# 4ment/physher

Hardware: AMD Instinct MI355X
Metric: lnL+gradient evals/sec, 1000-taxon GTR+G4 fp64, 1e6 site patterns (higher is better)
Workload: dtype f64

## Files before the change

include/physher_amd.h:

```cpp
#ifndef PHYSHER_AMD_H
#define PHYSHER_AMD_H

#include <stddef.h>
#include <stdint.h>

#ifdef __cplusplus
extern "C" {
#endif

typedef struct phyamd_engine phyamd_engine;

enum {
	PHYAMD_OK = 0,
	PHYAMD_EINVAL = -1,
	PHYAMD_EDEVICE = -2,
	PHYAMD_ENOMEM = -3,
	PHYAMD_EUNSUPPORTED = -4
};

enum { PHYAMD_RESCALE_NEVER = 0, PHYAMD_RESCALE_ALWAYS = 1, PHYAMD_RESCALE_AUTO = 2 };

enum {
	PHYAMD_GRAD_FOLD_ROOT_FREQS = 1,
	PHYAMD_GRAD_COMPAT_SCALED = 2
// ... 91 lines not shown
                                         double *replicate_lnl );
typedef struct { int32_t items, chunks, replicate_chunks, lower_slots; int64_t scratch_bytes; double ms; } phyamd_site_lnl_profile;
int phyamd_get_site_lnl_profile(phyamd_engine *e, phyamd_site_lnl_profile *out);
int phyamd_synchronize(phyamd_engine *e);

int phyamd_get_pattern_log_likelihoods(phyamd_engine *e, double *out );
int phyamd_get_partials(phyamd_engine *e, int node, int upper, double *out);
int phyamd_get_node_matrices(phyamd_engine *e, int node, int derivative, double *out );
int phyamd_post_order_parks(int32_t tip_count, const int32_t *left , const int32_t *right, int32_t root, int32_t second_slot,
                            int32_t *out , int32_t capacity);
#define PHYAMD_PRE_ORDER_COLUMNS 30
int phyamd_pre_order_schedule(int32_t tip_count, const int32_t *left , const int32_t *right, int32_t root, int32_t form,
                              int32_t *out , int32_t capacity, int32_t *hbm_slots);
int phyamd_post_order_slots(int32_t tip_count, const int32_t *left , const int32_t *right, int32_t root,
                            int32_t *out , int32_t capacity, int32_t *slots);
int phyamd_is_rescaling(phyamd_engine *e);
int phyamd_set_rescaling(phyamd_engine *e, int policy);
int phyamd_set_keep_partials(phyamd_engine *e, int on);

typedef struct {
	double matrices_ms, lower_ms, upper_ms, reduce_ms;
	int32_t lower_launches, upper_launches;
	int64_t device_bytes;
	int32_t tiles;
} phyamd_profile;
int phyamd_set_reduction_levels(phyamd_engine *e, int levels);
int phyamd_set_profiling(phyamd_engine *e, int on);
int phyamd_get_profile(phyamd_engine *e, phyamd_profile *out);

#ifdef __cplusplus
// ... 4 lines not shown
```

physher_amd/_lib.py:

```python
from __future__ import annotations

import ctypes as C
import os

_HERE = os.path.dirname(os.path.abspath(__file__))
LIB_PATH = os.environ.get("PHYAMD_LIB") or os.path.join(_HERE, "libphysher_amd.so")

ABI_VERSION = 5

OK, EINVAL, EDEVICE, ENOMEM, EUNSUPPORTED = 0, -1, -2, -3, -4
RESCALE_NEVER, RESCALE_ALWAYS, RESCALE_AUTO = 0, 1, 2
GRAD_FOLD_ROOT_FREQS, GRAD_COMPAT_SCALED = 1, 2


class Config(C.Structure):
    _fields_ = [
        ("tip_count", C.c_int32), ("pattern_count", C.c_int32), ("state_count", C.c_int32),
        ("category_count", C.c_int32), ("device", C.c_int32), ("rescale", C.c_int32),
        ("max_device_bytes", C.c_int64), ("stream", C.c_void_p),
    ]


class Profile(C.Structure):
    _fields_ = [
# ... 84 lines not shown
    ("phyamd_site_rate_posteriors", C.c_int, [_P, _P, _P]),
    ("phyamd_branch_hessian", C.c_int, [_P, C.c_int, _P, _P, _P]),
    ("phyamd_get_hessian_profile", C.c_int, [_P, C.POINTER(HessianProfile)]),
    ("phyamd_get_general_profile", C.c_int, [_P, C.POINTER(GeneralProfile)]),
    ("phyamd_gradient_batch_weights", C.c_int, [_P, C.c_int, C.c_int32, _P, _P, _P, _P]),
    ("phyamd_get_weight_batch_profile", C.c_int, [_P, C.POINTER(WeightBatchProfile)]),
    ("phyamd_pattern_log_likelihoods_trees", C.c_int, [_P, C.c_int, C.c_int32, _P, _P, _P, _P, _P, _P, C.c_int32, _P, _P]),
    ("phyamd_get_site_lnl_profile", C.c_int, [_P, C.POINTER(SiteLnlProfile)]),
    ("phyamd_synchronize", C.c_int, [_P]),
    ("phyamd_get_pattern_log_likelihoods", C.c_int, [_P, _P]),
    ("phyamd_get_partials", C.c_int, [_P, C.c_int, C.c_int, _P]),
    ("phyamd_get_node_matrices", C.c_int, [_P, C.c_int, C.c_int, _P]),
    ("phyamd_post_order_parks", C.c_int, [C.c_int32, _P, _P, C.c_int32, C.c_int32, _P, C.c_int32]),
    ("phyamd_post_order_slots", C.c_int, [C.c_int32, _P, _P, C.c_int32, _P, C.c_int32, _P]),
    ("phyamd_pre_order_schedule", C.c_int, [C.c_int32, _P, _P, C.c_int32, C.c_int32, _P, C.c_int32, _P]),
    ("phyamd_is_rescaling", C.c_int, [_P]),
    ("phyamd_set_rescaling", C.c_int, [_P, C.c_int]),
    ("phyamd_set_keep_partials", C.c_int, [_P, C.c_int]),
    ("phyamd_set_reduction_levels", C.c_int, [_P, C.c_int]),
    ("phyamd_set_profiling", C.c_int, [_P, C.c_int]),
    ("phyamd_get_profile", C.c_int, [_P, C.POINTER(Profile)]),
    ("phyamd_store", C.c_int, [_P]),
    ("phyamd_restore", C.c_int, [_P]),
    ("phyamd_compress_patterns", C.c_int, [C.c_int, C.c_int32, C.c_int64, _P, _P, C.POINTER(C.c_int32), _P, _P]),
]

_lib = None


def load():
# ... 21 lines not shown
```

physher_amd/csrc/phyamd_abi.inc:

```

#include <condition_variable>
#include <functional>
#include <mutex>
#include <thread>

namespace {

class ShardWorkers {
public:
	explicit ShardWorkers(int n) : done_(0), generation_(0), stop_(false) {
		for (int i = 0; i < n; i++) threads_.emplace_back([this, i] { loop(i); });
	}
	~ShardWorkers() {
		{
			std::lock_guard<std::mutex> lk(m_);
			stop_ = true;
			generation_++;
		}
		cv_.notify_all();
		for (auto &t : threads_) t.join();
	}
	void run(const std::function<void(int)> &fn) {
		std::unique_lock<std::mutex> lk(m_);
		fn_ = &fn;
// ... 820 lines not shown
			rec[18] = o.carry_out;
			const int kl = o.kind_left, kr = o.kind_right;
			const int rows[10] = {o.left, o.right, kl >= CH_CHERRY ? o.lt0 : -1, kl >= CH_CHERRY ? o.lt1 : -1, kl == CH_CHERRY_TIP ? o.linner : -1,
			                      kl == CH_CHERRY_TIP ? o.lt2 : -1, kr >= CH_CHERRY ? o.rt0 : -1, kr >= CH_CHERRY ? o.rt1 : -1,
			                      kr == CH_CHERRY_TIP ? o.rinner : -1, kr == CH_CHERRY_TIP ? o.rt2 : -1};
			for (int j = 0; j < 10; j++)
				if (rows[j] >= 0) q[nq++] = rows[j];
		}
		rec[17] = (is_cut_root[rec[2]] ? 1 : 0) | (is_cut_root[rec[3]] ? 2 : 0);
		rec[19] = nq;
		std::memcpy(out + (size_t)i * W, rec, sizeof(rec));
	}
	return (int)ops.size();
}

int phyamd_is_rescaling(phyamd_engine *g) {
	CHECK_GROUP(g);
	int any = 0;
	for (Shard *s : g->shards) any |= shard_is_rescaling(s);
	return any;
}

int phyamd_get_profile(phyamd_engine *g, phyamd_profile *out) {
	CHECK_GROUP(g);
	if (!out) return fail(PHYAMD_EINVAL, "null out");
	int rc;
	if ((rc = shard_get_profile(g->shards[0], out))) return rc;
	for (int i = 1; i < group_size(g); i++) {
		phyamd_profile p;
		if ((rc = shard_get_profile(g->shards[i], &p))) return rc;
// ... 12 lines not shown
```

physher_amd/csrc/phyamd_launch.inc:

```

size_t gen_image_doubles(const Shard *e) {
	return e->S == 20 ? MatImage<2, 5>::SIZE : e->S == 60 ? MatImage<4, 15>::SIZE : MatImage<4, 16>::SIZE;
}

template <int RT, int KT>
void launch_matrix_images(Shard *e, int count, const double *src, double *dst, const double *rowscale) {
	hipLaunchKernelGGL((k_matrix_images<RT, KT>), dim3(count), dim3(256), 0, e->stream, e->S, src, dst, rowscale);
}

void build_matrix_images(Shard *e, int count, const double *src, double *dst, const double *rowscale = nullptr) {
	if (e->S == 20) launch_matrix_images<2, 5>(e, count, src, dst, rowscale);
	else if (e->S == 60) launch_matrix_images<4, 15>(e, count, src, dst, rowscale);
	else launch_matrix_images<4, 16>(e, count, src, dst, rowscale);
}

int update_matrices(Shard *e) {
	if (e->generic && e->state.qimg_dirty && e->have_Q && e->have_freqs) {
		build_matrix_images(e, 1, e->d_Q, e->d_imgs + (size_t)e->N * e->C * gen_image_doubles(e));
		build_matrix_images(e, 1, e->d_Q, e->d_imgs + ((size_t)e->N * e->C + 1) * gen_image_doubles(e), e->d_freqs);
		HIP_TRY(hipGetLastError());
		q_images_rebuilt(e);
	}
	if (!e->state.matrices_dirty) return PHYAMD_OK;
	if (e->have_eigen) {
// ... 390 lines not shown
	if (v.scale < 0) return fail(PHYAMD_EDEVICE, "streamed walk: the stored lowers hold the %s form, which no %s post-order pass writes", form_name(e->lower_form), SCALE ? "rescaled" : "plain");
	const bool exp2 = v.scale == 2, tf = v.tf;
	if (exp2 && (rc = e->d_uexp.ensure(std::max<size_t>(1, upper_slots_held(e)) * e->C * e->P))) return rc;
	const int waves = SCALE && !exp2 ? e->C : STREAM_WAVES;
	const size_t lds = (size_t)STREAM_LDS_PER_WAVE * waves + (exp2 ? (size_t)waves * STREAM_PARK_SLOTS * WAVE * sizeof(int) : SCALE ? (size_t)4 * e->C * WAVE * sizeof(double) : 0);
	const dim3 grid_x(SCALE && !exp2 ? (unsigned)nb : (unsigned)((nb + STREAM_WAVES - 1) / STREAM_WAVES) * e->C), block(WAVE, waves);
	hipLaunchKernelGGL(k_op_tables, dim3(nops, e->C), dim3(64), 0, e->stream, nops, e->C, (const int *)e->d_stream_op_tips, (const int *)e->d_stream_op_deep,
	                   (const int *)e->d_stream_site_tab, e->d_mats, FOLD ? e->d_Q : e->d_Qpi, reinterpret_cast<double *>(e->d_optab.get()));
	const int subtrees = (int)e->sched.walk_chunk_off.size() - 2;
	for (int phase = 0; phase < (subtrees > 0 ? 2 : 1); phase++) {
		const bool amb = e->stream_ambiguous;
		auto *kernel = exp2 ? (amb ? k_upper4_stream<FOLD, 2, true, true> : k_upper4_stream<FOLD, 2, false, true>)
		             : SCALE ? (amb ? k_upper4_stream<FOLD, 1, true, false> : k_upper4_stream<FOLD, 1, false, false>)
		             : tf    ? (amb ? k_upper4_stream<FOLD, 0, true, true> : k_upper4_stream<FOLD, 0, false, true>)
		                     : (amb ? k_upper4_stream<FOLD, 0, true, false> : k_upper4_stream<FOLD, 0, false, false>);
		hipLaunchKernelGGL(kernel, dim3(grid_x.x, phase ? subtrees : 1), block, lds, e->stream, (const StreamDesc *)e->d_stream_ops, (const StreamChunk *)e->d_stream_chunks,
		                   (const int *)e->d_walk_chunk_off, phase, nops, e->P, e->C, nb, (const uint32_t *)e->d_mstream, e->mstride, (const double *)e->d_lower, e->d_upper,
		                   (const double *)e->d_mats, (const char *)e->d_optab, (const double *)(FOLD ? e->d_Q : e->d_Qpi), (const double *)e->d_freqs, (const double *)e->d_wl,
		                   e->d_gslab, R, (const double *)e->d_props, (const double *)e->d_weights, e->xcd_map, (const int *)e->d_lexp, e->d_uexp, (const int *)e->d_Eroot);
	}
	HIP_TRY(hipGetLastError());
	e->prof.upper_launches = subtrees > 0 ? 2 : 1;
	e->grad_blocks = nb;
	e->slab_walk_order = true;
	return PHYAMD_OK;
}

void bisect_blocks(int lo, int hi, int levels, std::vector<int> &bounds) {
	if (levels == 0) {
		bounds.push_back(lo);
		return;
// ... 404 lines not shown
```

physher_amd/csrc/phyamd_schedule.inc:

```

int bind_device(Shard *e) {
	HIP_TRY(hipSetDevice(e->device));
	return PHYAMD_OK;
}

size_t node_partial_doubles(const Shard *e) { return (size_t)e->C * e->S * (e->generic ? e->Pp : e->P); }
size_t lower_slots(const Shard *e) { return e->d_lower.size() / node_partial_doubles(e); }
size_t upper_slots_held(const Shard *e) { return e->d_upper.size() / node_partial_doubles(e); }

int ensure_lower_storage(Shard *e) {
	const size_t need = (size_t)std::max(1, e->sched.core_count) * (e->two_slots ? 2 : 1);
	if (lower_slots(e) >= need) return PHYAMD_OK;
	e->d_lower.release();
	e->d_lscale.release();
	return e->d_lower.ensure(need * node_partial_doubles(e));
}

void refresh_op_cores(Schedule &s) {
	for (std::vector<NodeOp> *ops : {&s.lower_ops, &s.upper_ops, &s.walk_lower_ops, &s.walk_upper_ops, &s.walk_chunk_ops, &s.walk_lower_chunk_ops})
		for (NodeOp &op : *ops) {
			op.core_parent = s.core_index[op.parent];
			op.core_left = s.core_index[op.left];
			op.core_right = s.core_index[op.right];
		}
// ... 9 lines not shown
		HIP_TRY(hipMemcpyAsync(e->d_tiptab + (size_t)e->T * e->C * 64, e->sched.deep_host.data(), e->sched.deep_host.size() * sizeof(DeepDesc), hipMemcpyHostToDevice,
		                       e->stream));
	if (e->sched.walking || e->sched.gen_walking) {
		if ((rc = e->d_walk_lower_ops.ensure(e->N)) || (rc = e->d_walk_upper_ops.ensure(e->N))) return rc;
		HIP_TRY(hipMemcpyAsync(e->d_walk_lower_ops, e->sched.walk_lower_ops.data(), e->sched.walk_lower_ops.size() * sizeof(NodeOp), hipMemcpyHostToDevice, e->stream));
		HIP_TRY(hipMemcpyAsync(e->d_walk_upper_ops, e->sched.walk_upper_ops.data(), e->sched.walk_upper_ops.size() * sizeof(NodeOp), hipMemcpyHostToDevice, e->stream));
	}
	if (e->sched.walking) {
		if ((rc = e->d_walk_chunk_ops.ensure(e->N)) || (rc = e->d_walk_chunk_off.ensure((size_t)e->N + 2))) return rc;
		HIP_TRY(hipMemcpyAsync(e->d_walk_chunk_ops, e->sched.walk_chunk_ops.data(), e->sched.walk_chunk_ops.size() * sizeof(NodeOp), hipMemcpyHostToDevice, e->stream));
		HIP_TRY(hipMemcpyAsync(e->d_walk_chunk_off, e->sched.walk_chunk_off.data(), e->sched.walk_chunk_off.size() * sizeof(int), hipMemcpyHostToDevice, e->stream));
		if ((rc = e->d_walk_lower_chunk_ops.ensure(e->N)) || (rc = e->d_walk_lower_chunk_off.ensure((size_t)e->N + 2))) return rc;
		HIP_TRY(hipMemcpyAsync(e->d_walk_lower_chunk_ops, e->sched.walk_lower_chunk_ops.data(), e->sched.walk_lower_chunk_ops.size() * sizeof(NodeOp), hipMemcpyHostToDevice, e->stream));
		HIP_TRY(hipMemcpyAsync(e->d_walk_lower_chunk_off, e->sched.walk_lower_chunk_off.data(), e->sched.walk_lower_chunk_off.size() * sizeof(int), hipMemcpyHostToDevice, e->stream));
		if (stream_possible(e)) {
			build_stream_tables(e->sched, StreamGeometry{e->P, e->C, (size_t)e->nblk_walk_upper * e->G * WAVE}, &e->stream_tab);
			if ((rc = e->d_stream_ops.ensure(e->N)) || (rc = e->d_stream_chunks.ensure((size_t)e->N + 2)) || (rc = e->d_stream_row_entries.ensure((size_t)e->N * 32)) ||
			    (rc = e->d_stream_site_tab.ensure((size_t)e->N * 16)) || (rc = e->d_stream_qnode.ensure(e->N)) || (rc = e->d_stream_op_tips.ensure((size_t)e->N * 12)) ||
			    (rc = e->d_stream_flag.ensure(1)) || (rc = e->d_stream_op_deep.ensure(e->N)))
				return rc;
			HIP_TRY(hipMemcpyAsync(e->d_stream_op_tips, e->stream_tab.op_tips.data(), e->stream_tab.op_tips.size() * sizeof(int), hipMemcpyHostToDevice, e->stream));
			HIP_TRY(hipMemcpyAsync(e->d_stream_op_deep, e->stream_tab.op_deep.data(), e->stream_tab.op_deep.size() * sizeof(int), hipMemcpyHostToDevice, e->stream));
			HIP_TRY(hipMemcpyAsync(e->d_stream_ops, e->stream_tab.desc.data(), e->stream_tab.desc.size() * sizeof(StreamDesc), hipMemcpyHostToDevice, e->stream));
			HIP_TRY(hipMemcpyAsync(e->d_stream_chunks, e->stream_tab.chunks.data(), e->stream_tab.chunks.size() * sizeof(StreamChunk), hipMemcpyHostToDevice, e->stream));
			HIP_TRY(hipMemcpyAsync(e->d_stream_row_entries, e->stream_tab.row_entries.data(), e->stream_tab.row_entries.size() * sizeof(int), hipMemcpyHostToDevice, e->stream));
			HIP_TRY(hipMemcpyAsync(e->d_stream_site_tab, e->stream_tab.site_tab.data(), e->stream_tab.site_tab.size() * sizeof(int), hipMemcpyHostToDevice, e->stream));
			HIP_TRY(hipMemcpyAsync(e->d_stream_qnode, e->stream_tab.qnode.data(), e->stream_tab.qnode.size() * sizeof(int), hipMemcpyHostToDevice, e->stream));
			if ((rc = e->d_lstream_ops.ensure(e->N)) || (rc = e->d_lstream_chunks.ensure((size_t)e->N + 2))) return rc;
			HIP_TRY(hipMemcpyAsync(e->d_lstream_ops, e->stream_tab.lower_desc.data(), e->stream_tab.lower_desc.size() * sizeof(LowerDesc), hipMemcpyHostToDevice, e->stream));
			HIP_TRY(hipMemcpyAsync(e->d_lstream_chunks, e->stream_tab.lower_chunks.data(), e->stream_tab.lower_chunks.size() * sizeof(LowerChunk), hipMemcpyHostToDevice, e->stream));
		}
	}
	std::vector<uint8_t> valid((size_t)e->N * e->C, 1);
	for (int c = 0; c < e->C; c++) valid[(size_t)e->root * e->C + c] = 0;
	HIP_TRY(hipMemcpyAsync(e->d_row_valid, valid.data(), valid.size(), hipMemcpyHostToDevice, e->stream));
	HIP_TRY(hipStreamSynchronize(e->stream));
	return PHYAMD_OK;
}

// ... 27 lines not shown
```

physher_amd/csrc/phyamd_shard.inc:

```

enum class LowerForm { Reference, Carried, CarriedExp2 };

struct ScheduleCounts { int core_count, upper_slots, widest; };

struct Shard {
	phyamd_config cfg{};
	DeviceBudget mem;
	DeviceBudget tile_mem{&mem};
	int T = 0, N = 0, P = 0, S = 0, C = 0, root = -1;
	int G = 1;
	bool generic = false;
	int Pp = 0;
	int nblk_root = 0;
	int nblk_lower = 0;
	int nblk_walk = 0, nblk_walk_upper = 0;
	int lower_walk_slots[2] = {0, 0};
	int gen_slots[3][2] = {};
	int lnl_blocks = 0;
	int grad_blocks = 0;
	size_t gpart_row = 0;
	struct State {
		bool all_dirty = true;
		std::vector<int> changed;
		bool force_root = false;
// ... 67 lines not shown
	int device = 0;
	hipStream_t stream = nullptr;
	bool own_stream = false;

	std::vector<int32_t> left, right;
	std::vector<double> lengths, model, freqs, rates, props;
	std::vector<double> lengths_sent;
	std::vector<uint8_t> explicit_host;
	bool have_topology = false, have_lengths = false, have_eigen = false, have_freqs = false, have_rates = false, have_weights = false;
	std::vector<uint8_t> tip_set;
	bool scaling_on = false;
	LowerForm lower_form = LowerForm::Reference;
	bool reference_form_only = false;
	bool exp2_on = true, tform_on = true;
	bool lower_park2_on = true;
	DeviceArray<int> d_lexp{&tile_mem}, d_uexp{&tile_mem}, d_Ec{&tile_mem}, d_Eroot{&tile_mem};
	bool keep_partials = false;
	bool profiling = false;
	bool prof_pending = false, prof_with_upper = false;

	Schedule sched;
	Schedule sched_spare;
	StreamTables stream_tab;
	ScheduleCounts scaled_counts{0, 0, 1};
	bool have_scaled_counts = false;
	bool fusion_enabled = true;

	DeviceArray<uint8_t> d_tipmask{&tile_mem};
	DeviceArray<unsigned long long> d_tipsets{&mem};
	std::vector<unsigned long long> tipsets_host;
// ... 238 lines not shown
```

physher_amd/csrc/phyamd_shard_api.inc:

```

ScheduleCounts schedule_counts(const Schedule &s) {
	ScheduleCounts c{s.core_count, std::max(s.upper_slots, s.walk_upper_slots), 1};
	for (size_t i = 0; i + 1 < s.lower_level_off.size(); i++) c.widest = std::max(c.widest, s.lower_level_off[i + 1] - s.lower_level_off[i]);
	for (size_t i = 0; i + 1 < s.upper_level_off.size(); i++) c.widest = std::max(c.widest, s.upper_level_off[i + 1] - s.upper_level_off[i]);
	return c;
}

double tile_working_set(const Shard *e, double p, bool exact, const ScheduleCounts &k) {
	const double pp = e->S == 4 ? p : std::ceil(p / 16.0) * 16.0, npd = (double)e->C * e->S * pp;
	const double per_pattern = (double)e->T * p + 8.0 * p * (3.0 + (e->S == 4 ? 0.0 : (double)e->C));
	const bool may_scale = e->cfg.rescale != PHYAMD_RESCALE_NEVER, exponents = may_scale && e->S == 4 && e->exp2_on;
	if (!exact) return 8.0 * (exponents ? 1.125 : 1.0) * ((e->S == 4 ? 0.5 : 1.6) * (double)(e->N - e->T) * npd + 2.0 * npd) + per_pattern;
	double doubles = (double)(std::max(1, k.core_count) + std::max(1, k.upper_slots)) * npd;
	if (may_scale) doubles += (double)std::max(1, k.core_count) * p + (e->S == 4 ? 0.0 : 5.0 * k.widest * e->C * p);
	if (exponents) doubles += 0.5 * ((double)(std::max(1, k.core_count) + std::max(1, k.upper_slots) + 1) * e->C * p + p);
	if (e->S == 4) doubles += (double)e->C * p;
	doubles += (double)e->N * e->C * (p / (WAVE * std::max(1, 4 / e->C)) + 1.0);
	if (e->S == 4) doubles += 2.0 * e->N * (p / (WAVE * PPT_UPPER) + 19.0) + 0.5 * p / 64.0;
	return 8.0 * doubles + per_pattern;
}

double tile_working_set(const Shard *e, double p, bool exact) {
	const double now = tile_working_set(e, p, exact, schedule_counts(e->sched));
	return e->have_scaled_counts ? std::max(now, tile_working_set(e, p, exact, e->scaled_counts)) : now;
// ... 135 lines not shown
	if ((rc = choose_tiles(e, false))) return bail(rc);
	if (cfg->stream) e->stream = (hipStream_t)cfg->stream;
	else {
		hipError_t err = hipStreamCreateWithFlags(&e->stream, hipStreamNonBlocking);
		if (err != hipSuccess) return bail(fail(PHYAMD_EDEVICE, "hipStreamCreate: %s", hipGetErrorString(err)));
		e->own_stream = true;
	}
	e->scaling_on = cfg->rescale == PHYAMD_RESCALE_ALWAYS;
	if (const char *env = std::getenv("PHYAMD_FUSE")) e->fusion_enabled = std::atoi(env) != 0;
	if (const char *env = std::getenv("PHYAMD_WALK")) e->walk_enabled = std::atoi(env) != 0;
	if (const char *env = std::getenv("PHYAMD_GEN_FUSION")) e->generic_fusion = std::atoi(env) != 0;
	if (const char *env = std::getenv("PHYAMD_XCD_MAP")) e->xcd_map = std::atoi(env) != 0;
	if (const char *env = std::getenv("PHYAMD_SCALE_EXP2")) e->exp2_on = std::atoi(env) != 0;
	if (const char *env = std::getenv("PHYAMD_STREAM_TFORM")) e->tform_on = std::atoi(env) != 0;
	if (const char *env = std::getenv("PHYAMD_LOWER_PARK2")) e->lower_park2_on = std::atoi(env) != 0;
	e->generic = e->S != 4;
	e->tip_set.assign(e->T, 0);
	e->tip_empty.assign(e->T, 0);
	e->mem.spare = &e->batch_mem;
	e->batch_max_patterns = BATCH_MAX_PATTERNS;
	if (const char *env = std::getenv("PHYAMD_BATCH_MAX_PATTERNS")) e->batch_max_patterns = std::atoi(env);
	if (const char *env = std::getenv("PHYAMD_BATCH_TRACE")) e->batch_trace = std::atoi(env) != 0;
	e->explicit_host.assign(e->N, 0);
	const size_t msz = (size_t)e->N * e->C * e->S * e->S;
	if (e->generic && ((rc = e->d_tipsets.ensure(256)) || (rc = e->d_imgs.ensure(((size_t)e->N * e->C + 2) * gen_image_doubles(e))))) return bail(rc);
	if (e->S == 20 && GenFuse<2>::QP) {
		if ((rc = e->d_qp_mats.ensure((size_t)e->T * e->C * e->S * e->S)) || (rc = e->d_qp_imgs.ensure((size_t)e->T * e->C * gen_image_doubles(e)))) return bail(rc);
	}
	if ((rc = e->d_mats.ensure(msz)) || (rc = e->d_dmats.ensure(msz)) || (rc = e->d_model.ensure((size_t)e->S + 2 * e->S * e->S)) ||
	    (rc = e->d_Q.ensure((size_t)e->S * e->S)))
// ... 895 lines not shown
```

physher_amd/csrc/phyamd_tree_schedule.h:

```cpp
#ifndef PHYAMD_TREE_SCHEDULE_H
#define PHYAMD_TREE_SCHEDULE_H

#include <algorithm>
#include <cstdarg>
#include <cstdint>
#include <cstdio>
#include <string>
#include <utility>
#include <vector>

#include "phyamd_types.h"

struct TreeRef {
	int T;
	const int32_t *left, *right;
	int root;
};

inline std::string schedule_error(const char *fmt, ...) {
	char buf[512];
	va_list ap;
	va_start(ap, fmt);
	vsnprintf(buf, sizeof buf, fmt, ap);
	va_end(ap);
// ... 525 lines not shown
		sc.walk_lower_ops.reserve(tree.T - 1);
		sc.walk_upper_ops.reserve(tree.T - 1);
		b.walk_post_order();
		b.walk_pre_order();
		if (sc.walking) {
			chunk_pre_order(sc);
			chunk_post_order(sc);
		}
	}
	return std::string();
}

struct StreamGeometry {
	int P, C;
	size_t mstride;
};

struct StreamTables {
	std::vector<StreamOp> ops;
	std::vector<StreamDesc> desc;
	int P = 0;
	size_t mstride = 0;
	std::vector<StreamChunk> chunks;
	std::vector<LowerDesc> lower_desc;
	std::vector<LowerChunk> lower_chunks;
	std::vector<int> row_entries;
	std::vector<int> site_tab;
	std::vector<int> qnode;
	std::vector<int> op_tips;
	std::vector<int> op_deep;
	int words = 0, R = 0;
};

struct MaskPacker {
	std::vector<int> &rows;
	int row = -1, used = 32, entries = 8;
	explicit MaskPacker(std::vector<int> &r) : rows(r), row((int)r.size() / 8 - 1) {}
	void add(const int *tips, int &out_row, int &out_shift) {
		int span = 0, n = 0;
		for (int j = 0; j < 6; j++)
			if (tips[j] >= 0) {
				span = j + 1;
				n++;
			}
		const int bits = 1 + 4 * span;
// ... 285 lines not shown
			const bool last = i + 1 == en;
			const int sn = last ? 0 : sop[sc.walk_lower_chunk_ops[i + 1].parent];
			d.nx_block = sn;
			int first = 0;
			const int count = last ? 0 : fresh_rows(i + 1, first);
			d.nx_words = (int64_t)first * row_bytes;
			d.flags |= count << 14;
			d.flags |= (first & 3) << 12;
			d.flags |= (last ? 0 : ((pieces[i + 1] & 2) ? 1 : 0)) << 24;
			d.flags |= (last ? 0 : (pieces[i + 1] & 1)) << 25;
		}
	}
	t.words = (int)t.row_entries.size() / 8;
}

inline void build_stream_tables(const Schedule &sc, const StreamGeometry &g, StreamTables *out) {
	stream_pre_order(sc, g, *out);
	stream_post_order(sc, g, *out);
}


inline int build_batch_ops(int T, const int32_t *left, const int32_t *right, int root, std::vector<BatchOp> *ops, bool park_all = false) {
	const int N = 2 * T - 1;
	std::vector<int> size(N, 1), order;
	{
		std::vector<int> stack{root};
		while (!stack.empty()) {
			const int n = stack.back();
			stack.pop_back();
			order.push_back(n);
			if (n >= T) {
				stack.push_back(left[n]);
				stack.push_back(right[n]);
// ... 99 lines not shown
```

physher_amd/csrc/phyamd_types.h:

```cpp
#ifndef PHYAMD_TYPES_H
#define PHYAMD_TYPES_H

#include <cstddef>
#include <cstdint>

constexpr int WAVE = 64;

enum { CH_TIP = 0, CH_CORE = 1, CH_DEEP = 2, CH_CHERRY = 3, CH_CHERRY_TIP = 4 };

struct DeepDesc {
	int32_t kind_left, left, lt0, lt1, lt2, linner;
	int32_t kind_right, right, rt0, rt1, rt2, rinner;
};

struct NodeOp {
	int32_t parent;
	int32_t left, right;
	int32_t upper_slot_parent;
	int32_t upper_slot_left, upper_slot_right;
	int32_t core_parent, core_left, core_right;
	int32_t kind_left, kind_right;
	int32_t lt0, lt1, lt2, linner;
	int32_t rt0, rt1, rt2, rinner;
	int32_t carry_in;
// ... 1 lines not shown
	int32_t lds_park;
};

constexpr int WALK_CHUNKS = 3;

struct BatchOp {
	int32_t node, left, right;
	int32_t carry;
	int32_t src, dst_left, dst_right;
	int32_t pad;
};
enum { BATCH_NONE = -1, BATCH_CARRY = -2, BATCH_ROOT = -3, BATCH_GHOST = -4 };

enum { HK_TIP = 0, HK_CHERRY = 1, HK_CHERRY_TIP = 2 };
enum { SU_CARRY = 0, SU_LDS = 1, SU_U = 2, SU_ROOT = 3 };

struct StreamOp {
	int32_t flags;
	int32_t parent;
	int32_t slot_parent, slot_left, slot_right;
	int32_t nx_mask_word;
	int32_t nx_a, nx_b;
	int32_t lnode, la[10];
	int32_t rnode, ra[10];
	int32_t nx_u;
	int32_t wsh;
};
static_assert(sizeof(StreamOp) == 128, "one StreamOp = 32 dwords");

struct StreamDesc {
// ... 39 lines not shown
```

physher_amd/csrc/phyamd_walk4s.inc:

```


__global__ __launch_bounds__(256) void k_build_mask_stream(int rows, int P, size_t mstride, const int *__restrict__ row_entries, const uint8_t *__restrict__ tipmask,
                                                           uint32_t *__restrict__ mstream, int *__restrict__ flags) {
	const size_t k = (size_t)blockIdx.x * 256 + threadIdx.x;
	if (k >= mstride) return;
	bool bad = false, amb = false;
	for (int w = blockIdx.y; w < rows; w += gridDim.y) {
		uint32_t v = 0;
		for (int j = 0; j < 8; j++) {
			const int ent = row_entries[w * 8 + j];
			if (ent < 0) continue;
			const int t = ent & 0xFFFFF, pos = (ent >> 20) & 31, fpos = (ent >> 25) & 31;
			const uint32_t m = (k < (size_t)P ? tipmask[(size_t)t * P + k] : 0xFu) & 0xFu;
			const uint32_t code = m == 1 ? 0 : m == 2 ? 1 : m == 4 ? 2 : m == 8 ? 3 : (m == 15 || m == 0) ? 4 : m == 3 ? 5 : m < 8 ? m + 1 : m;
			bad |= m == 0;
			if (code >= 5) {
				amb = true;
				v |= 1u << fpos;
			}
			v |= code << pos;
		}
		mstream[(size_t)w * mstride + k] = v;
	}
	if (bad || amb) atomicOr(flags, (bad ? 1 : 0) | (amb ? 2 : 0));
// ... 102 lines not shown
	template <int A, int R, bool FIRST = false>
	__device__ __forceinline__ void add_tip(const d4 &u, const d4 &qb) {
		put<A, R, FIRST>(dot4(u, qb));
	}
};

template <int SIDE, bool KEEP_BN>
__device__ __forceinline__ d4 s_fringe_message(const SX &x, int kind, int node, int inner, unsigned w, d4 &bn) {
	d4 p = mul4(x.site_tip<SIDE, 0>(w), x.site_tip<SIDE, 1>(w));
	if (kind == CH_CHERRY_TIP) {
		const d4 inner_message = matvec4_opt<false>(x.M(inner), p);
		if (KEEP_BN) bn = inner_message;
		p = mul4(inner_message, x.site_tip<SIDE, 2>(w));
	}
	return matvec4_opt<false>(x.M(node), p);
}

template <int SIDE, bool FIRST2, bool KEEP_BN, typename SS>
__device__ __forceinline__ void s_descend(const SX &x, SS &ss, int kind, int node, int inner, const d4 &u, unsigned w, const d4 &bn_kept) {
	d4 a2 = matvec4_opt<false>(x.M(node), u);
	if (kind == CH_CHERRY_TIP) {
		const d4 bn = KEEP_BN ? bn_kept : matvec4_opt<false>(x.M(inner), mul4(x.site_tip<SIDE, 0>(w), x.site_tip<SIDE, 1>(w)));
		const d4 un = mul4(a2, x.site_tip<SIDE, 2>(w));
		ss.template add<SIDE, 3>(un, bn);
		ss.template add_tip<2, SIDE, FIRST2>(mul4(a2, bn), x.site_tip_q<SIDE, 2>(w));
		a2 = matvec4_opt<false>(x.M(inner), un);
	}
	ss.template add_tip<SIDE, 1>(mul4(a2, x.site_tip<SIDE, 1>(w)), x.site_tip_q<SIDE, 0>(w));
	ss.template add_tip<SIDE, 2>(mul4(a2, x.site_tip<SIDE, 0>(w)), x.site_tip_q<SIDE, 1>(w));
}
// ... 211 lines not shown
		} else if (usrc == SU_U) {
			ea = eU;
			a = matvec4_opt<false>(x.M(op.parent), U);
			if (!SCALE && !valid) a = d4{0., 0., 0., 0.};
		}
		else a = FOLD ? d4{wl * freqs[0], wl * freqs[1], wl * freqs[2], wl * freqs[3]} : d4{wl, wl, wl, wl};
		d4 bl, br, bnl, bnr;
		if (KEEP_BN) {
			any_value(bnl);
			any_value(bnr);
		}
		if (kl == CH_CORE) bl = TF ? own_registers(A) : matvec4_opt<false>(x.M(op.lnode), A);
		else if (kl == CH_TIP) bl = x.site_tip<0, 0>(wL);
		else if (kl == CH_DEEP)
			bl = matvec4_opt<false>(x.M(op.lnode), mul4(s_half<0, 0>(x, (fl >> 16) & 3, op.lm[0], op.lm[1], wL), s_half<0, 3>(x, (fl >> 18) & 3, op.lm[2], op.lm[3], wL)));
		else bl = s_fringe_message<0, KEEP_BN>(x, kl, op.lnode, op.lm[4], wL, bnl);
		if (kr == CH_CORE) br = TF ? own_registers(B) : matvec4_opt<false>(x.M(op.rnode), B);
		else if (kr == CH_TIP) br = x.site_tip<1, 0>(wR);
		else if (kr == CH_DEEP)
			br = matvec4_opt<false>(x.M(op.rnode), mul4(s_half<1, 0>(x, (fl >> 20) & 3, op.rm[0], op.rm[1], wR), s_half<1, 3>(x, (fl >> 22) & 3, op.rm[2], op.rm[3], wR)));
		else br = s_fringe_message<1, KEEP_BN>(x, kr, op.rnode, op.rm[4], wR, bnr);
		const int e_bl = EXP2 && kl == CH_CORE ? eA : 0, e_br = EXP2 && kr == CH_CORE ? eB : 0;
		__builtin_amdgcn_s_setprio(3);
		unsigned nw0 = 0, nw1 = 0;
		if (i + 1 < op_end) fetch_block(i + 1, (fl >> 24) & 1);
		if (nxw > 0) nw0 = word_at(op.nx_words);
		if (nxw > 1) nw1 = word_at(op.nx_words + ((fl >> 25) & 1 ? (int64_t)0 : (int64_t)mrow));
		if (fl & (1 << 26)) A = lower_at(op.nx_a);
		if (fl & (1 << 27)) B = lower_at(op.nx_b);
		if (fl & (1 << 28)) U = upper_at(op.nx_u);
		if (EXP2) {
			if (fl & (1 << 26)) eA = *reinterpret_cast<const int *>(lexp_c + (op.nx_a >> 3) + eoff);
			if (fl & (1 << 27)) eB = *reinterpret_cast<const int *>(lexp_c + (op.nx_b >> 3) + eoff);
			if (fl & (1 << 28)) eU = *reinterpret_cast<const int *>(uexp_c + (op.nx_u >> 3) + eoff);
		}
		__builtin_amdgcn_s_setprio(0);
		ul = mul4(a, br);
// ... 32 lines not shown
			park[ps + WAVE] = dv2{v.z, v.w};
			if (EXP2) pexp[(STREAM_PARK_SLOTS > 1 ? (fl >> 6) & 1 : 0) * WAVE] = pk == 1 ? e_l : e_r;
		}
		if ((fl & (1 << 29)) && valid) store_upper_at(op.st_left, ul);
		if ((fl & (1 << 30)) && valid) store_upper_at(op.st_right, ur);
		if (EXP2) {
			if ((fl & (1 << 29)) && valid) *reinterpret_cast<int *>(uexp_c + (op.st_left >> 3) + eoff) = e_l;
			if ((fl & (1 << 30)) && valid) *reinterpret_cast<int *>(uexp_c + (op.st_right >> 3) + eoff) = e_r;
		}
		if (kl == CH_TIP) ss.template add_tip<0, 0, true>(ul_terms, x.site_tip_q<0, 0>(wL));
		else ss.template add<0, 0, true>(ul_terms, bl);
		if (kr == CH_TIP) ss.template add_tip<1, 0, true>(ur_terms, x.site_tip_q<1, 0>(wR));
		else ss.template add<1, 0, true>(ur_terms, br);
		if (kl == CH_CHERRY_TIP) {
			s_descend<0, true, KEEP_BN>(x, ss, CH_CHERRY_TIP, op.lnode, op.lm[4], ul_terms, wL, bnl);
			if (kr >= CH_CHERRY) s_descend<1, false, KEEP_BN>(x, ss, kr, op.rnode, op.rm[4], ur_terms, wR, bnr);
			prev_tot = fold_sites<true>(ss.acc0, ss.acc1, ss.acc2);
		} else if (kr == CH_CHERRY_TIP) {
			if (kl == CH_CHERRY) s_descend<0, false, KEEP_BN>(x, ss, CH_CHERRY, op.lnode, op.lm[4], ul_terms, wL, bnl);
			s_descend<1, true, KEEP_BN>(x, ss, CH_CHERRY_TIP, op.rnode, op.rm[4], ur_terms, wR, bnr);
			prev_tot = fold_sites<true>(ss.acc0, ss.acc1, ss.acc2);
		} else {
			if (kl == CH_CHERRY) s_descend<0, false, KEEP_BN>(x, ss, CH_CHERRY, op.lnode, op.lm[4], ul_terms, wL, bnl);
			if (kr == CH_CHERRY) s_descend<1, false, KEEP_BN>(x, ss, CH_CHERRY, op.rnode, op.rm[4], ur_terms, wR, bnr);
			prev_tot = fold_sites<false>(ss.acc0, ss.acc1, 0.0);
		}
		prev_off = soff;
		w0 = nw0;
		w1 = nw1;
		e_ul = e_l;
	}
// ... 147 lines not shown
				carry = d4{carry.x / m, carry.y / m, carry.z / m, carry.w / m};
				sfc += log(m);
			}
		}
		if (TF && op.self) carry = matvec4_opt<false>(x.M(op.self), carry);
		if (fl & (1 << 10)) {
			parked = carry;
			sfp = sfc;
			efp = efc;
		}
		if (PARK2 && (fl & (1 << 26))) {
			parked2 = carry;
			sfp2 = sfc;
			efp2 = efc;
		}
		have_prev = !(fl & (1 << 11));
		prev_store = op.store;
		prev_ls = op.ls_store;
	}
	if (have_prev) store_result(prev_store, carry);
	if (XCH && have_prev && c == 0 && valid) *reinterpret_cast<double *>(lscale_k + prev_ls) = sfc;
	if (EXP2 && have_prev && valid) *exp_at(prev_ls) = efc;
	if (with_root && valid) {
		Lc[(size_t)c * P + k] = props[c] * (freqs[0] * carry.x + freqs[1] * carry.y + freqs[2] * carry.z + freqs[3] * carry.w);
		if (EXP2) Ec[(size_t)c * P + k] = efc;
	}
}

__global__ __launch_bounds__(64) void k_root_finish64(int P, int C, const double *__restrict__ Lc, const double *__restrict__ weights, double *__restrict__ pattern_lk,
                                                     double *__restrict__ w_over_L, double *__restrict__ lnl_part, const double *__restrict__ lscale_root,
                                                     const int *__restrict__ Ec, int *__restrict__ Eroot) {
// ... 47 lines not shown
```

Baseline: 36.55.

## Elide stores of core-plus-fringe lower partials and recompute them in the upper stream

Adds a schedule pass that finds lower-pass nodes whose children are one core child and one tip or cherry, and whose parent is in the same chunk. For these nodes the lower walk skips writing the partial to memory. The upper stream kernel instead rebuilds the message from the stored core child and the fringe sibling, using new sibling kinds. This cuts HBM writes and reads of whole partial arrays in exchange for extra matvecs and more complex descriptor tables. A plain descriptor copy is kept for the non-tform path, and the feature is on by default with an env override.

```diff
diff --git a/include/physher_amd.h b/include/physher_amd.h
--- a/include/physher_amd.h
+++ b/include/physher_amd.h
@@ -129,6 +129,8 @@
                               int32_t *out , int32_t capacity, int32_t *hbm_slots);
 int phyamd_post_order_slots(int32_t tip_count, const int32_t *left , const int32_t *right, int32_t root,
                             int32_t *out , int32_t capacity, int32_t *slots);
+int phyamd_stream_elisions(int32_t tip_count, const int32_t *left , const int32_t *right, int32_t root,
+                           int32_t *out , int32_t capacity);
 int phyamd_is_rescaling(phyamd_engine *e);
 int phyamd_set_rescaling(phyamd_engine *e, int policy);
 int phyamd_set_keep_partials(phyamd_engine *e, int on);
diff --git a/physher_amd/_lib.py b/physher_amd/_lib.py
--- a/physher_amd/_lib.py
+++ b/physher_amd/_lib.py
@@ -122,6 +122,7 @@
     ("phyamd_post_order_parks", C.c_int, [C.c_int32, _P, _P, C.c_int32, C.c_int32, _P, C.c_int32]),
     ("phyamd_post_order_slots", C.c_int, [C.c_int32, _P, _P, C.c_int32, _P, C.c_int32, _P]),
     ("phyamd_pre_order_schedule", C.c_int, [C.c_int32, _P, _P, C.c_int32, C.c_int32, _P, C.c_int32, _P]),
+    ("phyamd_stream_elisions", C.c_int, [C.c_int32, _P, _P, C.c_int32, _P, C.c_int32]),
     ("phyamd_is_rescaling", C.c_int, [_P]),
     ("phyamd_set_rescaling", C.c_int, [_P, C.c_int]),
     ("phyamd_set_keep_partials", C.c_int, [_P, C.c_int]),
diff --git a/physher_amd/csrc/phyamd_abi.inc b/physher_amd/csrc/phyamd_abi.inc
--- a/physher_amd/csrc/phyamd_abi.inc
+++ b/physher_amd/csrc/phyamd_abi.inc
@@ -858,6 +858,23 @@
 	return (int)ops.size();
 }
 
+int phyamd_stream_elisions(int32_t tip_count, const int32_t *left, const int32_t *right, int32_t root, int32_t *out, int32_t capacity) {
+	if (tip_count < 2) return fail(PHYAMD_EINVAL, "tip_count must be >= 2 (got %d)", tip_count);
+	if (!left || !right) return fail(PHYAMD_EINVAL, "null left or right");
+	if (capacity < 0 || (capacity > 0 && !out)) return fail(PHYAMD_EINVAL, "null out with capacity %d", capacity);
+	Schedule sched;
+	StreamTables stream_tab;
+	const std::string err = build_schedule(TreeRef{tip_count, left, right, root}, ScheduleOptions{}, &sched);
+	if (!err.empty()) return fail(PHYAMD_EINVAL, "%s", err.c_str());
+	build_stream_tables(sched, StreamGeometry{1, 1, WAVE, true}, &stream_tab);
+	const std::vector<StreamElision> &el = stream_tab.elisions;
+	for (int i = 0; i < (int)el.size() && i < capacity; i++) {
+		const int32_t rec[8] = {el[i].node, el[i].parent, el[i].stored, el[i].sibling, el[i].sibling_kind, el[i].source, el[i].side, el[i].chunk};
+		std::memcpy(out + (size_t)i * 8, rec, sizeof(rec));
+	}
+	return (int)el.size();
+}
+
 int phyamd_is_rescaling(phyamd_engine *g) {
 	CHECK_GROUP(g);
 	int any = 0;
diff --git a/physher_amd/csrc/phyamd_launch.inc b/physher_amd/csrc/phyamd_launch.inc
--- a/physher_amd/csrc/phyamd_launch.inc
+++ b/physher_amd/csrc/phyamd_launch.inc
@@ -428,7 +428,9 @@
 		             : SCALE ? (amb ? k_upper4_stream<FOLD, 1, true, false> : k_upper4_stream<FOLD, 1, false, false>)
 		             : tf    ? (amb ? k_upper4_stream<FOLD, 0, true, true> : k_upper4_stream<FOLD, 0, false, true>)
 		                     : (amb ? k_upper4_stream<FOLD, 0, true, false> : k_upper4_stream<FOLD, 0, false, false>);
-		hipLaunchKernelGGL(kernel, dim3(grid_x.x, phase ? subtrees : 1), block, lds, e->stream, (const StreamDesc *)e->d_stream_ops, (const StreamChunk *)e->d_stream_chunks,
+		const bool plain = !tf && !e->stream_tab.plain_desc.empty();
+		hipLaunchKernelGGL(kernel, dim3(grid_x.x, phase ? subtrees : 1), block, lds, e->stream,
+		                   (const StreamDesc *)e->d_stream_ops + (plain ? e->stream_tab.desc.size() : 0), (const StreamChunk *)e->d_stream_chunks + (plain ? e->stream_tab.chunks.size() : 0),
 		                   (const int *)e->d_walk_chunk_off, phase, nops, e->P, e->C, nb, (const uint32_t *)e->d_mstream, e->mstride, (const double *)e->d_lower, e->d_upper,
 		                   (const double *)e->d_mats, (const char *)e->d_optab, (const double *)(FOLD ? e->d_Q : e->d_Qpi), (const double *)e->d_freqs, (const double *)e->d_wl,
 		                   e->d_gslab, R, (const double *)e->d_props, (const double *)e->d_weights, e->xcd_map, (const int *)e->d_lexp, e->d_uexp, (const int *)e->d_Eroot);
diff --git a/physher_amd/csrc/phyamd_schedule.inc b/physher_amd/csrc/phyamd_schedule.inc
--- a/physher_amd/csrc/phyamd_schedule.inc
+++ b/physher_amd/csrc/phyamd_schedule.inc
@@ -47,8 +47,9 @@
 		HIP_TRY(hipMemcpyAsync(e->d_walk_lower_chunk_ops, e->sched.walk_lower_chunk_ops.data(), e->sched.walk_lower_chunk_ops.size() * sizeof(NodeOp), hipMemcpyHostToDevice, e->stream));
 		HIP_TRY(hipMemcpyAsync(e->d_walk_lower_chunk_off, e->sched.walk_lower_chunk_off.data(), e->sched.walk_lower_chunk_off.size() * sizeof(int), hipMemcpyHostToDevice, e->stream));
 		if (stream_possible(e)) {
-			build_stream_tables(e->sched, StreamGeometry{e->P, e->C, (size_t)e->nblk_walk_upper * e->G * WAVE}, &e->stream_tab);
-			if ((rc = e->d_stream_ops.ensure(e->N)) || (rc = e->d_stream_chunks.ensure((size_t)e->N + 2)) || (rc = e->d_stream_row_entries.ensure((size_t)e->N * 32)) ||
+			build_stream_tables(e->sched, StreamGeometry{e->P, e->C, (size_t)e->nblk_walk_upper * e->G * WAVE, e->stream_elide_on}, &e->stream_tab);
+			if ((rc = e->d_stream_ops.ensure((size_t)2 * e->N)) || (rc = e->d_stream_chunks.ensure((size_t)2 * e->N + 4)) ||
+			    (rc = e->d_stream_row_entries.ensure(std::max((size_t)e->N * 32, e->stream_tab.row_entries.size()))) ||
 			    (rc = e->d_stream_site_tab.ensure((size_t)e->N * 16)) || (rc = e->d_stream_qnode.ensure(e->N)) || (rc = e->d_stream_op_tips.ensure((size_t)e->N * 12)) ||
 			    (rc = e->d_stream_flag.ensure(1)) || (rc = e->d_stream_op_deep.ensure(e->N)))
 				return rc;
@@ -56,6 +57,12 @@
 			HIP_TRY(hipMemcpyAsync(e->d_stream_op_deep, e->stream_tab.op_deep.data(), e->stream_tab.op_deep.size() * sizeof(int), hipMemcpyHostToDevice, e->stream));
 			HIP_TRY(hipMemcpyAsync(e->d_stream_ops, e->stream_tab.desc.data(), e->stream_tab.desc.size() * sizeof(StreamDesc), hipMemcpyHostToDevice, e->stream));
 			HIP_TRY(hipMemcpyAsync(e->d_stream_chunks, e->stream_tab.chunks.data(), e->stream_tab.chunks.size() * sizeof(StreamChunk), hipMemcpyHostToDevice, e->stream));
+			if (!e->stream_tab.plain_desc.empty()) {
+				HIP_TRY(hipMemcpyAsync(e->d_stream_ops + e->stream_tab.desc.size(), e->stream_tab.plain_desc.data(), e->stream_tab.plain_desc.size() * sizeof(StreamDesc),
+				                       hipMemcpyHostToDevice, e->stream));
+				HIP_TRY(hipMemcpyAsync(e->d_stream_chunks + e->stream_tab.chunks.size(), e->stream_tab.plain_chunks.data(),
+				                       e->stream_tab.plain_chunks.size() * sizeof(StreamChunk), hipMemcpyHostToDevice, e->stream));
+			}
 			HIP_TRY(hipMemcpyAsync(e->d_stream_row_entries, e->stream_tab.row_entries.data(), e->stream_tab.row_entries.size() * sizeof(int), hipMemcpyHostToDevice, e->stream));
 			HIP_TRY(hipMemcpyAsync(e->d_stream_site_tab, e->stream_tab.site_tab.data(), e->stream_tab.site_tab.size() * sizeof(int), hipMemcpyHostToDevice, e->stream));
 			HIP_TRY(hipMemcpyAsync(e->d_stream_qnode, e->stream_tab.qnode.data(), e->stream_tab.qnode.size() * sizeof(int), hipMemcpyHostToDevice, e->stream));
diff --git a/physher_amd/csrc/phyamd_shard.inc b/physher_amd/csrc/phyamd_shard.inc
--- a/physher_amd/csrc/phyamd_shard.inc
+++ b/physher_amd/csrc/phyamd_shard.inc
@@ -105,6 +105,7 @@
 	bool reference_form_only = false;
 	bool exp2_on = true, tform_on = true;
 	bool lower_park2_on = true;
+	bool stream_elide_on = true;
 	DeviceArray<int> d_lexp{&tile_mem}, d_uexp{&tile_mem}, d_Ec{&tile_mem}, d_Eroot{&tile_mem};
 	bool keep_partials = false;
 	bool profiling = false;
diff --git a/physher_amd/csrc/phyamd_shard_api.inc b/physher_amd/csrc/phyamd_shard_api.inc
--- a/physher_amd/csrc/phyamd_shard_api.inc
+++ b/physher_amd/csrc/phyamd_shard_api.inc
@@ -173,6 +173,7 @@
 	if (const char *env = std::getenv("PHYAMD_SCALE_EXP2")) e->exp2_on = std::atoi(env) != 0;
 	if (const char *env = std::getenv("PHYAMD_STREAM_TFORM")) e->tform_on = std::atoi(env) != 0;
 	if (const char *env = std::getenv("PHYAMD_LOWER_PARK2")) e->lower_park2_on = std::atoi(env) != 0;
+	if (const char *env = std::getenv("PHYAMD_STREAM_ELIDE")) e->stream_elide_on = std::atoi(env) != 0;
 	e->generic = e->S != 4;
 	e->tip_set.assign(e->T, 0);
 	e->tip_empty.assign(e->T, 0);
diff --git a/physher_amd/csrc/phyamd_tree_schedule.h b/physher_amd/csrc/phyamd_tree_schedule.h
--- a/physher_amd/csrc/phyamd_tree_schedule.h
+++ b/physher_amd/csrc/phyamd_tree_schedule.h
@@ -563,6 +563,14 @@
 struct StreamGeometry {
 	int P, C;
 	size_t mstride;
+	bool elide = false;
+};
+
+struct StreamElision {
+	int32_t node, parent, stored, sibling, sibling_kind;
+	int32_t source;
+	int32_t side;
+	int32_t chunk;
 };
 
 struct StreamTables {
@@ -578,6 +586,9 @@
 	std::vector<int> qnode;
 	std::vector<int> op_tips;
 	std::vector<int> op_deep;
+	std::vector<StreamDesc> plain_desc;
+	std::vector<StreamChunk> plain_chunks;
+	std::vector<StreamElision> elisions;
 	int words = 0, R = 0;
 };
 
@@ -893,9 +904,102 @@
 	t.words = (int)t.row_entries.size() / 8;
 }
 
+inline void stream_elide(const Schedule &sc, const StreamGeometry &g, StreamTables &t) {
+	t.plain_desc = t.desc;
+	t.plain_chunks = t.chunks;
+	t.elisions.clear();
+	const int n = (int)t.lower_desc.size(), ns = (int)t.ops.size(), N = (int)sc.parent.size();
+	if (n == 0 || ns == 0) return;
+	const std::vector<NodeOp> &lops = sc.walk_lower_chunk_ops;
+	std::vector<int> sop(N, -1), lop(N, -1), lchunk(n, 0);
+	for (int i = 0; i < ns; i++) sop[sc.walk_chunk_ops[i].parent] = i;
+	for (int i = 0; i < n; i++) lop[lops[i].parent] = i;
+	for (int k = 0; k + 1 < (int)sc.walk_lower_chunk_off.size(); k++)
+		for (int i = sc.walk_lower_chunk_off[k]; i < sc.walk_lower_chunk_off[k + 1]; i++) lchunk[i] = k;
+	std::vector<char> in_e(N, 0);
+	std::vector<int> elided_at((size_t)ns * 2, -1);
+	for (int i = 0; i < n; i++) {
+		const NodeOp &o = lops[i];
+		const int nd = o.parent, p = sc.parent[nd];
+		if (p < 0 || lop[p] < 0 || sop[p] < 0) continue;
+		const int kl = sc.node_kind[o.left], kr = sc.node_kind[o.right];
+		int s, f;
+		if (kl == CH_CORE && (kr == CH_TIP || kr == CH_CHERRY)) s = o.left, f = o.right;
+		else if (kr == CH_CORE && (kl == CH_TIP || kl == CH_CHERRY)) s = o.right, f = o.left;
+		else continue;
+		if (in_e[s] || lchunk[lop[p]] != lchunk[i]) continue;
+		const StreamOp &pu = t.ops[sop[p]];
+		const int side = pu.lnode == nd ? 0 : 1;
+		if ((side ? pu.rnode : pu.lnode) != nd || ((pu.flags >> (3 * side)) & 7) != CH_CORE) continue;
+		const int source = (t.lower_desc[lop[p]].flags >> (6 + 2 * side)) & 3;
+		if (source != 1 && source != 2) continue;
+		in_e[nd] = 1;
+		elided_at[(size_t)sop[p] * 2 + side] = (int)t.elisions.size();
+		t.elisions.push_back(StreamElision{nd, p, s, f, sc.node_kind[f], source, side, lchunk[i]});
+		t.lower_desc[i].flags |= 1 << 11;
+	}
+	if (t.elisions.empty()) return;
+	const int64_t plane_bytes = (int64_t)g.P * 4 * 8, array_bytes = plane_bytes * g.C, row_bytes = (int64_t)t.mstride * 4;
+	std::vector<int> chunk_of_start(ns, -1);
+	for (int k = 0; k + 1 < (int)sc.walk_chunk_off.size(); k++)
+		if (sc.walk_chunk_off[k] < sc.walk_chunk_off[k + 1]) chunk_of_start[sc.walk_chunk_off[k]] = k;
+	MaskPacker packer(t.row_entries);
+	for (int i = 0; i < ns; i++) {
+		if (elided_at[(size_t)i * 2] < 0 && elided_at[(size_t)i * 2 + 1] < 0) continue;
+		StreamDesc &d = t.desc[i];
+		int want[2] = {-1, -1};
+		for (int side = 0; side < 2; side++) {
+			if (elided_at[(size_t)i * 2 + side] < 0) continue;
+			const StreamElision &el = t.elisions[elided_at[(size_t)i * 2 + side]];
+			const NodeOp &o = lops[lop[el.node]];
+			const bool f_left = o.left == el.sibling;
+			int *tips = &t.op_tips[(size_t)i * 12 + 6 * side];
+			if (el.sibling_kind == CH_TIP) tips[0] = el.sibling;
+			else {
+				tips[0] = f_left ? o.lt0 : o.rt0;
+				tips[1] = f_left ? o.lt1 : o.rt1;
+			}
+			d.flags = (d.flags & ~(7 << (3 * side))) | (el.sibling_kind == CH_TIP ? SK_CORE_TIP : SK_CORE_CHERRY) << (3 * side);
+			(side ? d.rm : d.lm)[0] = el.sibling * g.C * 128;
+			want[side] = sc.core_index[el.stored];
+		}
+		int words = 0, first_word = -1, same_row = 0, wsh = 0;
+		for (int side = 0; side < 2; side++)
+			if (((d.flags >> (3 * side)) & 7) != CH_CORE) {
+				int row, shift;
+				packer.add(&t.op_tips[(size_t)i * 12 + 6 * side], row, shift);
+				if (words == 0) first_word = row;
+				else same_row = row == first_word;
+				wsh |= shift << (5 * words);
+				words++;
+			}
+		d.wsh = wsh;
+		const int two_pieces = ((d.flags >> 3) & 7) != CH_CORE;
+		if (chunk_of_start[i] >= 0) {
+			StreamChunk &ch = t.chunks[chunk_of_start[i]];
+			ch.mask_word = first_word;
+			ch.mask_words = words;
+			ch.same_row = same_row;
+			if (want[0] >= 0) ch.a = want[0];
+			if (want[1] >= 0) ch.b = want[1];
+		} else {
+			StreamDesc &pv = t.desc[i - 1];
+			pv.flags = (pv.flags & ~(3 << 14 | 1 << 24 | 1 << 25)) | words << 14 | two_pieces << 24 | same_row << 25;
+			pv.nx_words = (int64_t)first_word * row_bytes;
+			if (want[0] >= 0) pv.nx_a = (int64_t)want[0] * array_bytes;
+			if (want[1] >= 0) pv.nx_b = (int64_t)want[1] * array_bytes;
+		}
+	}
+	t.words = (int)t.row_entries.size() / 8;
+}
+
 inline void build_stream_tables(const Schedule &sc, const StreamGeometry &g, StreamTables *out) {
 	stream_pre_order(sc, g, *out);
 	stream_post_order(sc, g, *out);
+	out->plain_desc.clear();
+	out->plain_chunks.clear();
+	out->elisions.clear();
+	if (g.elide) stream_elide(sc, g, *out);
 }
 
 
diff --git a/physher_amd/csrc/phyamd_types.h b/physher_amd/csrc/phyamd_types.h
--- a/physher_amd/csrc/phyamd_types.h
+++ b/physher_amd/csrc/phyamd_types.h
@@ -39,6 +39,7 @@
 
 enum { HK_TIP = 0, HK_CHERRY = 1, HK_CHERRY_TIP = 2 };
 enum { SU_CARRY = 0, SU_LDS = 1, SU_U = 2, SU_ROOT = 3 };
+enum { SK_CORE_TIP = 5, SK_CORE_CHERRY = 6 };
 
 struct StreamOp {
 	int32_t flags;
diff --git a/physher_amd/csrc/phyamd_walk4s.inc b/physher_amd/csrc/phyamd_walk4s.inc
--- a/physher_amd/csrc/phyamd_walk4s.inc
+++ b/physher_amd/csrc/phyamd_walk4s.inc
@@ -140,6 +140,13 @@
 		p = mul4(inner_message, x.site_tip<SIDE, 2>(w));
 	}
 	return matvec4_opt<false>(x.M(node), p);
+}
+
+template <int SIDE>
+__device__ __forceinline__ d4 s_elided_message(const SX &x, int kind, int node, int fm, unsigned w, const d4 &ts) {
+	d4 unused;
+	const d4 mf = kind == SK_CORE_TIP ? x.site_tip<SIDE, 0>(w) : s_fringe_message<SIDE, false>(x, CH_CHERRY, fm, 0, w, unused);
+	return matvec4_opt<false>(x.M(node), mul4(mf, ts));
 }
 
 template <int SIDE, bool FIRST2, bool KEEP_BN, typename SS>
@@ -381,13 +388,15 @@
 		else if (kl == CH_TIP) bl = x.site_tip<0, 0>(wL);
 		else if (kl == CH_DEEP)
 			bl = matvec4_opt<false>(x.M(op.lnode), mul4(s_half<0, 0>(x, (fl >> 16) & 3, op.lm[0], op.lm[1], wL), s_half<0, 3>(x, (fl >> 18) & 3, op.lm[2], op.lm[3], wL)));
+		else if (TF && kl >= SK_CORE_TIP) bl = s_elided_message<0>(x, kl, op.lnode, op.lm[0], wL, A);
 		else bl = s_fringe_message<0, KEEP_BN>(x, kl, op.lnode, op.lm[4], wL, bnl);
 		if (kr == CH_CORE) br = TF ? own_registers(B) : matvec4_opt<false>(x.M(op.rnode), B);
 		else if (kr == CH_TIP) br = x.site_tip<1, 0>(wR);
 		else if (kr == CH_DEEP)
 			br = matvec4_opt<false>(x.M(op.rnode), mul4(s_half<1, 0>(x, (fl >> 20) & 3, op.rm[0], op.rm[1], wR), s_half<1, 3>(x, (fl >> 22) & 3, op.rm[2], op.rm[3], wR)));
+		else if (TF && kr >= SK_CORE_TIP) br = s_elided_message<1>(x, kr, op.rnode, op.rm[0], wR, B);
 		else br = s_fringe_message<1, KEEP_BN>(x, kr, op.rnode, op.rm[4], wR, bnr);
-		const int e_bl = EXP2 && kl == CH_CORE ? eA : 0, e_br = EXP2 && kr == CH_CORE ? eB : 0;
+		const int e_bl = EXP2 && (kl == CH_CORE || kl >= SK_CORE_TIP) ? eA : 0, e_br = EXP2 && (kr == CH_CORE || kr >= SK_CORE_TIP) ? eB : 0;
 		__builtin_amdgcn_s_setprio(3);
 		unsigned nw0 = 0, nw1 = 0;
 		if (i + 1 < op_end) fetch_block(i + 1, (fl >> 24) & 1);
@@ -450,7 +459,7 @@
 		else ss.template add<1, 0, true>(ur_terms, br);
 		if (kl == CH_CHERRY_TIP) {
 			s_descend<0, true, KEEP_BN>(x, ss, CH_CHERRY_TIP, op.lnode, op.lm[4], ul_terms, wL, bnl);
-			if (kr >= CH_CHERRY) s_descend<1, false, KEEP_BN>(x, ss, kr, op.rnode, op.rm[4], ur_terms, wR, bnr);
+			if (kr == CH_CHERRY || kr == CH_CHERRY_TIP) s_descend<1, false, KEEP_BN>(x, ss, kr, op.rnode, op.rm[4], ur_terms, wR, bnr);
 			prev_tot = fold_sites<true>(ss.acc0, ss.acc1, ss.acc2);
 		} else if (kr == CH_CHERRY_TIP) {
 			if (kl == CH_CHERRY) s_descend<0, false, KEEP_BN>(x, ss, CH_CHERRY, op.lnode, op.lm[4], ul_terms, wL, bnl);
@@ -628,7 +637,7 @@
 			sfp2 = sfc;
 			efp2 = efc;
 		}
-		have_prev = !(fl & (1 << 11));
+		have_prev = !(TF && (fl & (1 << 11)));
 		prev_store = op.store;
 		prev_ls = op.ls_store;
 	}
```

Measured after the change: 37.28, median of 6. 2.0% higher.
